# haesungpyun/seoul_tourism_recommendation_NGCF

Hardware: NVIDIA B200
Metric: ngcf_epoch_time_fwd_bwd_bpr (lower is better)
Workload: dtype f32

## Files before the change

seoul_tourism_recommendation_ngcf_b200/csrc/spmm.cu:

```cuda
#include "spmm_core.cuh"

namespace {

using namespace ngcf;

#ifndef NGCF_SPMM_THREADS
#define NGCF_SPMM_THREADS 64
#endif
constexpr int SP_THREADS = NGCF_SPMM_THREADS;
constexpr int SP_WARPS = SP_THREADS / 32;

struct TileSide {
    const TileInfo* tiles;
    const int32_t* rowptr;
    const int2* ent;
    const int32_t* row_key;
    const uint8_t* bits;
    const int2* cent;
    const int32_t* ccnt;
    float* Y;
    int64_t ldy;
};

struct SpmmArgs {
    TileSide rows, chunks;
    int n_chunk_tiles;
    const float* X;
    uint32_t ldx;
    int d;
    const float* addend;
    int64_t ld_add;
    const int32_t* slot;
    const float* gsum;
    int64_t ld_gsum;
    const int32_t* hub_of_row;
    const int32_t* hub_chunk_ptr;
    int32_t* hub_done;
    float* Yrows;
    int64_t ld_yrows;
    float drop_p;
    uint64_t seed;
    const uint64_t* seed_dev;
    int layer;
    int transposed;
    uint32_t row_off;
    unsigned long long* dbg;
    const uint32_t* tile_hubmask;
    int n_row_tiles;
    int add_mode;
    const int32_t* hub_rows;
    int n_hub;
};

__device__ __forceinline__ unsigned long long gtime_ns() {
    unsigned long long t;
    asm volatile("mov.u64 %0, %%globaltimer;" : "=l"(t));
    return t;
}
__device__ __forceinline__ void stamp_done(unsigned long long* dbg) {
    __syncthreads();
    if (threadIdx.x == 0) {
        unsigned smid;
        asm volatile("mov.u32 %0, %%smid;" : "=r"(smid));
        dbg[blockIdx.x * 4 + 2] = gtime_ns();
        dbg[blockIdx.x * 4 + 3] = smid;
    }
}

struct CtaSync {
    __device__ __forceinline__ void operator()() const { __syncthreads(); }
};

#ifndef NGCF_SPMM_CTAS
#define NGCF_SPMM_CTAS 20
#endif
template <int G>
__global__ void __launch_bounds__(SP_THREADS, NGCF_SPMM_CTAS) spmm_tile_kernel(SpmmArgs a) {
    __shared__ __align__(16) int2 ent_s[SP_TILE_ENT];
    __shared__ int rp_s[SP_TILE_ROWS + 1];
    __shared__ int hub_s[SP_TILE_ROWS];
    const int tid = threadIdx.x, lane = tid & 31, warp = tid >> 5;
    pdl_launch_dependents();
    if (a.dbg && tid == 0) a.dbg[blockIdx.x * 4 + 0] = gtime_ns();
    const bool chunk_side = (int)blockIdx.x < a.n_chunk_tiles;
    const TileSide& sd = chunk_side ? a.chunks : a.rows;
    const int t = chunk_side ? (int)blockIdx.x : (int)blockIdx.x - a.n_chunk_tiles;
    const int4 raw = *reinterpret_cast<const int4*>(sd.tiles + t);
    const TileInfo ti{raw.x, raw.y, raw.z, raw.w};
    const int nr = ti.r1 - ti.r0;
    if (tid < nr)
        hub_s[tid] = chunk_side ? a.hub_of_row[sd.row_key[ti.r0 + tid]] : (a.hub_of_row ? a.hub_of_row[ti.r0 + tid] : -1);
    pdl_wait();
    {
        DropArgs dr{a.drop_p, a.drop_p > 0.f ? ngcf_seed(a.seed, a.seed_dev) : 0ull, a.layer, a.transposed,
                    a.row_off, sd.bits};
        stage_tile<SP_THREADS>(ti, sd.rowptr, sd.ent, sd.row_key, dr, rp_s, ent_s, tid, CtaSync());
    }
    if (a.dbg && tid == 0) a.dbg[blockIdx.x * 4 + 1] = gtime_ns();

    if (chunk_side) {
        for (int i = warp; i < nr; i += SP_WARPS) {
            const int64_t chunk = ti.r0 + i;
            const int h = hub_s[i];
            if constexpr (G > 0) {
                const float4 acc = gather_row_vec<G>(ent_s, rp_s[i], rp_s[i + 1], a.X, a.ldx, a.d, lane);
                if (lane < G && lane * 4 < a.d) st_f4(sd.Y + chunk * sd.ldy + lane * 4, acc);
            } else {
                float acc[SC_MAXQ];
                gather_row_sc(ent_s, rp_s[i], rp_s[i + 1], a.X, a.ldx, a.d, lane, acc);
#pragma unroll
                for (int q = 0; q < SC_MAXQ; ++q)
                    if (lane + 32 * q < a.d) sd.Y[chunk * sd.ldy + lane + 32 * q] = acc[q];
            }
            __threadfence();
            __syncwarp();
            const int c0 = a.hub_chunk_ptr[h], c1 = a.hub_chunk_ptr[h + 1];
            int last = 0;
            if (lane == 0) last = (atomicAdd(a.hub_done + h, 1) + 1 == c1 - c0);
            last = __shfl_sync(FULL_MASK, last, 0);
            if (!last) continue;
            __threadfence();
            if (lane == 0) a.hub_done[h] = 0;
            const int64_t row = sd.row_key[chunk] ;
            const int s = a.slot ? a.slot[row] : -1;
            if constexpr (G > 0) {
                float4 sum = sum_partials_split<G>(sd.Y, c0, c1, a.d, lane);
                if (lane < G && lane * 4 < a.d) {
                    const int c = lane * 4;
                    if (a.addend) {
                        const float4 ad = ld_f4(a.addend + row * a.ld_add + c);
                        sum.x += ad.x; sum.y += ad.y; sum.z += ad.z; sum.w += ad.w;
                    }
                    if (s >= 0) {
                        const float4 gs = ld_f4(a.gsum + (int64_t)s * a.ld_gsum + c);
                        sum.x += gs.x; sum.y += gs.y; sum.z += gs.z; sum.w += gs.w;
                    }
                    st_f4(a.Yrows + row * a.ld_yrows + c, sum);
                }
            } else {
                float sum[SC_MAXQ];
                sum_partials_sc(sd.Y, c0, c1, a.d, lane, sum);
#pragma unroll
                for (int q = 0; q < SC_MAXQ; ++q) {
                    const int col = lane + 32 * q;
                    if (col < a.d) {
                        float r = sum[q];
                        if (a.addend) r += a.addend[row * a.ld_add + col];
                        if (s >= 0) r += a.gsum[(int64_t)s * a.ld_gsum + col];
                        a.Yrows[row * a.ld_yrows + col] = r;
                    }
                }
            }
        }
        if (a.dbg) stamp_done(a.dbg);
        return;
    }

    if constexpr (G > 0) {
        for (int i = warp; i < nr; i += SP_WARPS) {
            if (hub_s[i] >= 0) continue;
            const int64_t row = ti.r0 + i;
            const bool ok = lane < G && lane * 4 < a.d;
            float4 ad = make_float4(0.f, 0.f, 0.f, 0.f);
            int s = -1;
            if (ok && a.addend) ad = ld_f4(a.addend + row * a.ld_add + lane * 4);
            if (ok && a.slot) s = a.slot[row];
            float4 acc = gather_row_vec<G>(ent_s, rp_s[i], rp_s[i + 1], a.X, a.ldx, a.d, lane);
            if (ok) {
                acc.x += ad.x; acc.y += ad.y; acc.z += ad.z; acc.w += ad.w;
                if (s >= 0) {
                    const float4 gs = ld_f4(a.gsum + (int64_t)s * a.ld_gsum + lane * 4);
                    acc.x += gs.x; acc.y += gs.y; acc.z += gs.z; acc.w += gs.w;
                }
                st_f4(sd.Y + row * sd.ldy + lane * 4, acc);
            }
        }
    } else {
        for (int i = warp; i < nr; i += SP_WARPS) {
            if (hub_s[i] >= 0) continue;
            const int64_t row = ti.r0 + i;
            float acc[SC_MAXQ];
            gather_row_sc(ent_s, rp_s[i], rp_s[i + 1], a.X, a.ldx, a.d, lane, acc);
            const int s = a.slot ? a.slot[row] : -1;
#pragma unroll
            for (int q = 0; q < SC_MAXQ; ++q) {
                const int col = lane + 32 * q;
                if (col < a.d) {
                    float r = acc[q];
                    if (a.addend) r += a.addend[row * a.ld_add + col];
                    if (s >= 0) r += a.gsum[(int64_t)s * a.ld_gsum + col];
                    sd.Y[row * sd.ldy + col] = r;
                }
            }
        }
    }
    if (a.dbg) stamp_done(a.dbg);
}

__device__ __forceinline__ void red_add_f4(float* p, float4 v) {
    asm volatile("red.global.add.v4.f32 [%0], {%1, %2, %3, %4};" ::"l"(p), "f"(v.x), "f"(v.y), "f"(v.z), "f"(v.w) : "memory");
}

template <int G>
__global__ void __launch_bounds__(SP_THREADS, NGCF_SPMM_CTAS) spmm_stream_kernel(SpmmArgs a) {
    constexpr int NGRP = SP_THREADS / G;
    __shared__ __align__(16) int2 ent_s[SP_TILE_ENT];
    __shared__ __align__(16) float ysum[SP_TILE_ROWS * G * 4];
    __shared__ __align__(16) float pf[SP_THREADS * 4];
    __shared__ int rp_s[SP_TILE_ROWS + 1];
    __shared__ int first_row[NGRP];
    const int tid = threadIdx.x, lane = tid & 31, warp = tid >> 5;
    const int grp = tid / G, l = tid % G;
    pdl_launch_dependents();
    if (a.dbg && tid == 0) a.dbg[blockIdx.x * 4 + 0] = gtime_ns();
    const bool chunk_side = (int)blockIdx.x < a.n_chunk_tiles;
    const TileSide& sd = chunk_side ? a.chunks : a.rows;
    const int t = chunk_side ? (int)blockIdx.x : (int)blockIdx.x - a.n_chunk_tiles;
    const int4 raw = *reinterpret_cast<const int4*>(sd.tiles + t);
    const TileInfo ti{raw.x, raw.y, raw.z, raw.w};
    const int nr = ti.r1 - ti.r0;
    const uint32_t hubmask = (!chunk_side && a.tile_hubmask) ? a.tile_hubmask[t] : 0u;
#pragma unroll
    for (int i = tid; i < SP_TILE_ROWS * G; i += SP_THREADS) reinterpret_cast<float4*>(ysum)[i] = make_float4(0.f, 0.f, 0.f, 0.f);
    pdl_wait();
    int cnt;
    if (sd.ccnt) {
        cnt = sd.ccnt[t];
        for (int i = tid; i < cnt; i += SP_THREADS) ent_s[i] = ld_stream_i2(sd.cent + ti.e0 + i);
        __syncthreads();
    } else {
        cnt = ti.e1 - ti.e0;
        DropArgs dr{a.drop_p, a.drop_p > 0.f ? ngcf_seed(a.seed, a.seed_dev) : 0ull, a.layer, a.transposed,
                    a.row_off, sd.bits};
        stage_tile<SP_THREADS>(ti, sd.rowptr, sd.ent, sd.row_key, dr, rp_s, ent_s, tid, CtaSync());
    }
    if (a.dbg && tid == 0) a.dbg[blockIdx.x * 4 + 1] = gtime_ns();

    {
        const int per = (cnt + NGRP - 1) / NGRP;
        int j = min(grp * per, cnt);
        const int end = min(j + per, cnt);
        const char* xl = reinterpret_cast<const char*>(a.X + ((l * 4) < a.d ? l * 4 : 0));
        const uint32_t row_bytes = a.ldx * 4u;
        float* const pf_l = pf + grp * (G * 4) + l * 4;
        float* const ys_l = ysum + l * 4;
        float4 acc = make_float4(0.f, 0.f, 0.f, 0.f);
        int cur = -1, frow = -1;
        bool isfirst = true;
        auto step = [&](const int2 e, const float4 x) {
            const int lr = ent_lrow(e.x);
            if (lr != cur) {
                if (cur >= 0) {
                    st_f4(isfirst ? pf_l : ys_l + cur * (G * 4), acc);
                    if (isfirst) frow = cur;
                    isfirst = false;
                }
                acc = make_float4(0.f, 0.f, 0.f, 0.f);
                cur = lr;
            }
            const float w = __int_as_float(e.y);
            acc.x = fmaf(w, x.x, acc.x);
            acc.y = fmaf(w, x.y, acc.y);
            acc.z = fmaf(w, x.z, acc.z);
            acc.w = fmaf(w, x.w, acc.w);
        };
        for (; j + UNROLL <= end; j += UNROLL) {
            int2 e[UNROLL];
            float4 x[UNROLL];
#pragma unroll
            for (int u = 0; u < UNROLL; ++u) e[u] = ent_s[j + u];
#pragma unroll
            for (int u = 0; u < UNROLL; ++u)
                x[u] = ld_f4(reinterpret_cast<const float*>(xl + (uint64_t)ent_col(e[u].x) * row_bytes));
#pragma unroll
            for (int u = 0; u < UNROLL; ++u) step(e[u], x[u]);
        }
        if (j < end) {
            int2 e[UNROLL];
            float4 x[UNROLL];
#pragma unroll
            for (int u = 0; u < UNROLL; ++u) {
                e[u] = make_int2(0, 0);
                x[u] = make_float4(0.f, 0.f, 0.f, 0.f);
                if (j + u < end) {
                    e[u] = ent_s[j + u];
                    x[u] = ld_f4(reinterpret_cast<const float*>(xl + (uint64_t)ent_col(e[u].x) * row_bytes));
                }
            }
#pragma unroll
            for (int u = 0; u < UNROLL; ++u)
                if (j + u < end) step(e[u], x[u]);
        }
        if (cur >= 0) {
            st_f4(isfirst ? pf_l : ys_l + cur * (G * 4), acc);
            if (isfirst) frow = cur;
        }
        if (l == 0) first_row[grp] = frow;
    }
    __syncthreads();

    auto row_sum = [&](int i, int ll) {
        float4 y = ld_f4(ysum + i * (G * 4) + ll * 4);
#pragma unroll
        for (int q = 0; q < NGRP; ++q)
            if (first_row[q] == i) {
                const float4 p = ld_f4(pf + q * (G * 4) + ll * 4);
                y.x += p.x; y.y += p.y; y.z += p.z; y.w += p.w;
            }
        return y;
    };

    if (chunk_side) {
        const bool okc = l * 4 < a.d;
        for (int i = grp; i < nr; i += NGRP)
            if (okc) st_f4(sd.Y + (int64_t)(ti.r0 + i) * sd.ldy + l * 4, row_sum(i, l));
        if (a.dbg) stamp_done(a.dbg);
        return;
    }

    const bool ok = l * 4 < a.d;
    for (int i = grp; i < nr; i += NGRP) {
        if (((hubmask >> i) & 1u) || !ok) continue;
        const int64_t row = ti.r0 + i;
        float4 y = row_sum(i, l);
        const int s = a.slot ? a.slot[row] : -1;
        if (s >= 0) {
            const float4 gs = ld_f4(a.gsum + (int64_t)s * a.ld_gsum + l * 4);
            y.x += gs.x; y.y += gs.y; y.z += gs.z; y.w += gs.w;
        }
        float* dst = sd.Y + row * sd.ldy + l * 4;
        if (a.add_mode) red_add_f4(dst, y); else st_f4(dst, y);
    }
    if (a.dbg) stamp_done(a.dbg);
}

constexpr int HF_THREADS = 128;
template <int G>
__global__ void __launch_bounds__(HF_THREADS) hub_finish_kernel(SpmmArgs a) {
    constexpr int NGRP = HF_THREADS / G;
    __shared__ __align__(16) float gs[HF_THREADS * 4];
    pdl_launch_dependents();
    const int tid = threadIdx.x, g = tid / G, l = tid % G;
    const int h = blockIdx.x;
    const int c0 = a.hub_chunk_ptr[h], c1 = a.hub_chunk_ptr[h + 1];
    const int64_t row = a.hub_rows[h];
    pdl_wait();
    const bool ok = l * 4 < a.d;
    float* const dst = a.Yrows + row * a.ld_yrows + l * 4;
    float4 ad = make_float4(0.f, 0.f, 0.f, 0.f);
    int s = -1;
    if (g == 0 && ok) {
        if (a.add_mode) ad = ld_f4(dst);
        if (a.slot) s = a.slot[row];
    }
    float4 acc = make_float4(0.f, 0.f, 0.f, 0.f);
    if (ok) {
        const float* p = a.chunks.Y + l * 4;
        int c = c0 + g;
        for (; c + 3 * NGRP < c1; c += 4 * NGRP) {
            float4 x[4];
#pragma unroll
            for (int u = 0; u < 4; ++u) x[u] = __ldcg(reinterpret_cast<const float4*>(p + (int64_t)(c + u * NGRP) * a.d));
#pragma unroll
            for (int u = 0; u < 4; ++u) { acc.x += x[u].x; acc.y += x[u].y; acc.z += x[u].z; acc.w += x[u].w; }
        }
        for (; c < c1; c += NGRP) {
            const float4 x = __ldcg(reinterpret_cast<const float4*>(p + (int64_t)c * a.d));
            acc.x += x.x; acc.y += x.y; acc.z += x.z; acc.w += x.w;
        }
    }
    st_f4(gs + g * (G * 4) + l * 4, acc);
    __syncthreads();
    if (g == 0 && ok) {
        float4 sum = acc;
#pragma unroll
        for (int q = 1; q < NGRP; ++q) {
            const float4 v = ld_f4(gs + q * (G * 4) + l * 4);
            sum.x += v.x; sum.y += v.y; sum.z += v.z; sum.w += v.w;
        }
        if (a.add_mode) {
            sum.x += ad.x; sum.y += ad.y; sum.z += ad.z; sum.w += ad.w;
        }
        if (s >= 0) {
            const float4 gsv = ld_f4(a.gsum + (int64_t)s * a.ld_gsum + l * 4);
            sum.x += gsv.x; sum.y += gsv.y; sum.z += gsv.z; sum.w += gsv.w;
        }
        st_f4(dst, sum);
    }
}

struct BitsArgs {
    const TileInfo* tiles;
    const int32_t* rowptr;
    const int2* ent;
    const int32_t* row_key;
    float p;
    uint64_t seed;
    const uint64_t* seed_dev;
    int n_layers;
    uint32_t row_off;
    uint8_t* out_f;
    uint8_t* out_t;
};

constexpr int BITS_THREADS = 256;
constexpr int BITS_TILES = 8;
__global__ void __launch_bounds__(BITS_THREADS) dropout_bits_kernel(BitsArgs a, int n_tiles) {
    __shared__ int rp_s[BITS_TILES * SP_TILE_ROWS + 1];
    const int tid = threadIdx.x;
    const int t0 = blockIdx.x * BITS_TILES, t1 = min(t0 + BITS_TILES, n_tiles) - 1;
    const int4 first = *reinterpret_cast<const int4*>(a.tiles + t0);
    const int4 last = *reinterpret_cast<const int4*>(a.tiles + t1);
    const int r0 = first.x, nr = last.y - first.x, e0 = first.z, cnt = last.w - first.z;
    for (int i = tid; i <= nr; i += BITS_THREADS) rp_s[i] = a.rowptr[r0 + i] - e0;
    __syncthreads();
    const uint64_t seed = ngcf_seed(a.seed, a.seed_dev);
    for (int i = tid; i < cnt; i += BITS_THREADS) {
        const uint32_t c = ent_col(ld_stream_i2(a.ent + e0 + i).x);
        int lo = 0, hi = nr - 1;
        while (lo < hi) {
            const int mid = (lo + hi + 1) >> 1;
            if (rp_s[mid] <= i) lo = mid; else hi = mid - 1;
        }
        const uint32_t r = (uint32_t)(a.row_key ? a.row_key[r0 + lo] : r0 + lo) + a.row_off;
        if (a.out_f) a.out_f[e0 + i] = (uint8_t)node_keep_bits(a.p, seed, a.n_layers, r, c);
        if (a.out_t) a.out_t[e0 + i] = (uint8_t)node_keep_bits(a.p, seed, a.n_layers, c, r);
    }
}

struct KeyArgs {
    const TileInfo* tiles;
    const int32_t* rowptr;
    const int2* ent;
    const int32_t* row_key;
    uint32_t row_off;
    uint32_t* key_l;
    uint32_t* key_t;
};
__global__ void __launch_bounds__(BITS_THREADS) entry_keys_kernel(KeyArgs a, int n_tiles) {
    __shared__ int rp_s[BITS_TILES * SP_TILE_ROWS + 1];
    const int tid = threadIdx.x;
    const int t0 = blockIdx.x * BITS_TILES, t1 = min(t0 + BITS_TILES, n_tiles) - 1;
    const int4 first = *reinterpret_cast<const int4*>(a.tiles + t0);
    const int4 last = *reinterpret_cast<const int4*>(a.tiles + t1);
    const int r0 = first.x, nr = last.y - first.x, e0 = first.z, cnt = last.w - first.z;
    for (int i = tid; i <= nr; i += BITS_THREADS) rp_s[i] = a.rowptr[r0 + i] - e0;
    __syncthreads();
    for (int i = tid; i < cnt; i += BITS_THREADS) {
        const uint32_t c = ent_col(ld_stream_i2(a.ent + e0 + i).x);
        int lo = 0, hi = nr - 1;
        while (lo < hi) {
            const int mid = (lo + hi + 1) >> 1;
            if (rp_s[mid] <= i) lo = mid; else hi = mid - 1;
        }
        const uint32_t r = (uint32_t)(a.row_key ? a.row_key[r0 + lo] : r0 + lo) + a.row_off;
        a.key_l[e0 + i] = ngcf_node_key(r, c);
        a.key_t[e0 + i] = ngcf_node_key(c, r);
    }
}

constexpr int WS_PER = SP_TILE_ENT / 32;
static_assert(WS_PER * 32 == SP_TILE_ENT, "tile entries must be a multiple of the warp size");

struct CompactArgs {
    const TileInfo* tiles;
    const int2* ent;
    const int32_t* row_key;
    float p;
    uint64_t seed;
    const uint64_t* seed_dev;
    int n_layers;
    uint32_t row_off;
    const uint32_t* key_l;
    const uint32_t* key_t;
    int2* out_ent[2][NGCF_MAX_LAYERS];
    int32_t* out_cnt[2][NGCF_MAX_LAYERS];
};

constexpr int CW_WARPS = 4;
__global__ void __launch_bounds__(CW_WARPS * 32) compact_kernel(CompactArgs a, int n_tiles) {
    const int lane = threadIdx.x & 31;
    const int t = blockIdx.x * CW_WARPS + (threadIdx.x >> 5);
    if (t >= n_tiles) return;
    const int4 raw = *reinterpret_cast<const int4*>(a.tiles + t);
    const TileInfo ti{raw.x, raw.y, raw.z, raw.w};
    const int cnt = ti.e1 - ti.e0;
    const int K = a.n_layers;
    const bool want_l = a.out_ent[0][0] != nullptr, want_t = a.out_ent[1][0] != nullptr;
    int2 e[WS_PER];
    uint32_t kl[WS_PER], kt[WS_PER];
#pragma unroll
    for (int q = 0; q < WS_PER; ++q) {
        const int p = q * 32 + lane;
        e[q] = make_int2(0, 0);
        kl[q] = kt[q] = 0;
        if (p < cnt) {
            e[q] = ld_stream_i2(a.ent + ti.e0 + p);
            if (a.key_l) {
                if (want_l) kl[q] = a.key_l[ti.e0 + p];
                if (want_t) kt[q] = a.key_t[ti.e0 + p];
            }
        }
    }
    const uint64_t seed = ngcf_seed(a.seed, a.seed_dev);
    const uint32_t thr = ngcf_threshold16(a.p);
    uint32_t keep[WS_PER];
#pragma unroll
    for (int q = 0; q < WS_PER; ++q) {
        const int p = q * 32 + lane;
        keep[q] = 0;
        if (p < cnt) {
            if (!a.key_l) {
                const int lr = ent_lrow(e[q].x);
                const uint32_t r = (uint32_t)(a.row_key ? a.row_key[ti.r0 + lr] : ti.r0 + lr) + a.row_off;
                kl[q] = ngcf_node_key(r, ent_col(e[q].x));
                kt[q] = ngcf_node_key(ent_col(e[q].x), r);
            }
            if (want_l) keep[q] = node_keep_bits_key(thr, seed, K, kl[q]);
            if (want_t) keep[q] |= node_keep_bits_key(thr, seed, K, kt[q]) << K;
        }
    }
    const uint32_t below = (1u << lane) - 1u;
    for (int c = 0; c < 2 * K; ++c) {
        const int dir = c >= K, layer = dir ? c - K : c;
        int2* out = a.out_ent[dir][layer];
        if (!out) continue;
        int base = 0;
#pragma unroll
        for (int q = 0; q < WS_PER; ++q) {
            const bool k = (keep[q] >> c) & 1u;
            const uint32_t m = __ballot_sync(FULL_MASK, k);
            if (k) out[ti.e0 + base + __popc(m & below)] = e[q];
            base += __popc(m);
        }
        if (lane == 0) a.out_cnt[dir][layer][t] = base;
    }
}

template <int G>
int launch(const SpmmArgs& a, int n_ctas, bool stream, cudaStream_t st) {
    if (n_ctas <= 0) return NGCF_OK;
    if constexpr (G > 0) {
        if (stream) {
            NGCF_CUDA(ngcf_launch_pdl(spmm_stream_kernel<G>, dim3((unsigned)n_ctas), dim3(SP_THREADS), 0, st, a));
            NGCF_LAUNCH_OK("spmm_stream_kernel");
            if (a.n_hub > 0) {
                NGCF_CUDA(ngcf_launch_pdl(hub_finish_kernel<G>, dim3((unsigned)a.n_hub), dim3(HF_THREADS), 0, st, a));
                NGCF_LAUNCH_OK("hub_finish_kernel");
            }
            return NGCF_OK;
        }
    }
    NGCF_CUDA(ngcf_launch_pdl(spmm_tile_kernel<G>, dim3((unsigned)n_ctas), dim3(SP_THREADS), 0, st, a));
    NGCF_LAUNCH_OK("spmm_tile_kernel");
    return NGCF_OK;
}

int launch_any(const SpmmArgs& a, int n_ctas, bool vec, bool stream, cudaStream_t st) {
    if (!vec) return launch<0>(a, n_ctas, false, st);
    const int d4 = a.d / 4;
    if (d4 <= 1) return launch<1>(a, n_ctas, stream, st);
    if (d4 <= 2) return launch<2>(a, n_ctas, stream, st);
    if (d4 <= 4) return launch<4>(a, n_ctas, stream, st);
    if (d4 <= 8) return launch<8>(a, n_ctas, stream, st);
    if (d4 <= 16) return launch<16>(a, n_ctas, stream, st);
    return launch<32>(a, n_ctas, stream, st);
}

unsigned long long* g_spmm_dbg = nullptr;
unsigned long long* g_spmm_dbg_compact = nullptr;

inline bool aligned16(const void* p) { return (reinterpret_cast<uintptr_t>(p) & 15) == 0; }

}

extern "C" int ngcf_spmm_split_threshold(void) { return ngcf::SPLIT; }
extern "C" int ngcf_spmm_tile_rows(void) { return SP_TILE_ROWS; }
extern "C" int ngcf_spmm_tile_entries(void) { return SP_TILE_ENT; }

int ngcf_check_csr(const ngcf_csr* g, const char* who) {
    NGCF_REQUIRE(g != nullptr, "%s: csr descriptor is null", who);
    NGCF_REQUIRE(g->n_rows >= 0 && g->n_rows < ((int64_t)1 << 31), "%s: n_rows %lld", who, (long long)g->n_rows);
    NGCF_REQUIRE(g->n_rows == 0 || (g->rowptr && g->ent), "%s: rowptr/ent missing", who);
    NGCF_REQUIRE(g->n_hub >= 0 && g->n_chunks >= 0, "%s: negative hub counts", who);
    NGCF_REQUIRE(g->n_hub == 0 || (g->hub_of_row && g->hub_chunk_ptr && g->chunk_ptr && g->hub_ent && g->chunk_row),
                 "%s: hub arrays missing", who);
    return NGCF_OK;
}

extern "C" int ngcf_spmm(const ngcf_csr* g, const float* X, int64_t ldx, int d, const float* addend, int64_t ld_add,
                         const int32_t* slot, const float* gsum, int64_t ld_gsum, float* hub_partial, float drop_p,
                         uint64_t seed, const uint64_t* seed_dev, int layer, int transposed, int64_t row_offset,
                         const uint8_t* keep_bits, const int32_t* c_ent, const int32_t* c_cnt, float* Y, int64_t ldy,
                         void* stream) {
    int rc = ngcf_check_csr(g, "spmm");
    if (rc != NGCF_OK) return rc;
    NGCF_REQUIRE(X && Y, "spmm: null pointer");
    NGCF_REQUIRE(d > 0 && d <= NGCF_MAX_WIDTH, "spmm: width %d not in [1,%d]", d, NGCF_MAX_WIDTH);
    NGCF_REQUIRE(ldx >= d && ldy >= d && ldx < ((int64_t)1 << 31), "spmm: bad leading dimension");
    NGCF_REQUIRE(drop_p >= 0.f && drop_p < 1.f, "spmm: drop_p %f not in [0,1)", drop_p);
    NGCF_REQUIRE(layer >= 0 && layer < NGCF_MAX_LAYERS, "spmm: layer %d", layer);
    NGCF_REQUIRE(row_offset >= 0 && row_offset < ((int64_t)1 << 31), "spmm: row_offset %lld", (long long)row_offset);
    NGCF_REQUIRE(!slot || gsum, "spmm: slot given without gsum");
    NGCF_REQUIRE((c_ent == nullptr) == (c_cnt == nullptr), "spmm: c_ent and c_cnt go together");
    NGCF_REQUIRE(g->n_hub == 0 || hub_partial, "spmm: hub_partial scratch missing");
    NGCF_REQUIRE(g->n_tiles == 0 || g->tiles, "spmm: SpMM tiles missing");
    NGCF_REQUIRE(g->n_chunk_tiles == 0 || g->chunk_tiles, "spmm: chunk tiles missing");
    if (g->n_rows == 0) return NGCF_OK;
    cudaStream_t st = as_stream(stream);
    const bool vec = (d % 4 == 0) && (ldx % 4 == 0) && (ldy % 4 == 0) && aligned16(X) && aligned16(Y) &&
                     (!addend || (aligned16(addend) && ld_add % 4 == 0)) &&
                     (!slot || (aligned16(gsum) && ld_gsum % 4 == 0)) && (g->n_hub == 0 || aligned16(hub_partial));
    const bool hubs = g->n_hub > 0 && g->n_chunks > 0;
    const bool stream_k = vec && (!hubs || (g->tile_hubmask && g->hub_rows));
    NGCF_REQUIRE(stream_k || !c_ent, "spmm: compacted survivor lists need the streaming kernel (width %% 4 == 0)");
    NGCF_REQUIRE(stream_k || !hubs || g->hub_done, "spmm: hub_done counters missing");
    SpmmArgs a{};
    a.rows = TileSide{reinterpret_cast<const TileInfo*>(g->tiles), g->rowptr, reinterpret_cast<const int2*>(g->ent), nullptr,
                      keep_bits, reinterpret_cast<const int2*>(c_ent), c_cnt, Y, ldy};
    a.n_chunk_tiles = hubs ? g->n_chunk_tiles : 0;
    if (hubs)
        a.chunks = TileSide{reinterpret_cast<const TileInfo*>(g->chunk_tiles), g->chunk_ptr,
                            reinterpret_cast<const int2*>(g->hub_ent), g->chunk_row,
                            keep_bits ? keep_bits + g->rowptr_nnz : nullptr,
                            c_ent ? reinterpret_cast<const int2*>(c_ent) + g->rowptr_nnz : nullptr,
                            c_cnt ? c_cnt + g->n_tiles : nullptr, hub_partial, d};
    a.X = X; a.ldx = (uint32_t)ldx; a.d = d;
    a.addend = addend; a.ld_add = ld_add; a.slot = slot; a.gsum = gsum; a.ld_gsum = ld_gsum;
    a.drop_p = drop_p; a.seed = seed; a.seed_dev = seed_dev; a.layer = layer; a.transposed = transposed;
    a.row_off = (uint32_t)row_offset;
    a.dbg = g_spmm_dbg;
    a.hub_of_row = hubs ? g->hub_of_row : nullptr;
    a.hub_chunk_ptr = g->hub_chunk_ptr;
    a.hub_done = g->hub_done;
    a.Yrows = Y;
    a.ld_yrows = ldy;
    a.tile_hubmask = hubs ? g->tile_hubmask : nullptr;
    a.n_row_tiles = g->n_tiles;
    a.hub_rows = g->hub_rows;
    a.n_hub = hubs ? g->n_hub : 0;
    if (stream_k && addend) {
        if (addend != Y)
            NGCF_CUDA(cudaMemcpy2DAsync(Y, (size_t)ldy * sizeof(float), addend, (size_t)ld_add * sizeof(float),
                                        (size_t)d * sizeof(float), (size_t)g->n_rows, cudaMemcpyDeviceToDevice, st));
        a.add_mode = 1;
        a.addend = nullptr;
    }
    return launch_any(a, a.n_chunk_tiles + g->n_tiles, vec, stream_k, st);
}

extern "C" int ngcf_node_dropout_bits(const ngcf_csr* g, float drop_p, uint64_t seed, const uint64_t* seed_dev,
                                      int n_layers, int64_t row_offset, uint8_t* bits_as_L, uint8_t* bits_as_Lt,
                                      void* stream) {
    int rc = ngcf_check_csr(g, "node_dropout_bits");
    if (rc != NGCF_OK) return rc;
    NGCF_REQUIRE(drop_p > 0.f && drop_p < 1.f, "node_dropout_bits: drop_p %f not in (0,1)", drop_p);
    NGCF_REQUIRE(n_layers >= 1 && n_layers <= NGCF_MAX_LAYERS, "node_dropout_bits: n_layers %d", n_layers);
    NGCF_REQUIRE(bits_as_L || bits_as_Lt, "node_dropout_bits: no output");
    NGCF_REQUIRE(row_offset >= 0 && row_offset < ((int64_t)1 << 31), "node_dropout_bits: row_offset");
    cudaStream_t st = as_stream(stream);
    if (g->n_tiles > 0) {
        BitsArgs a{reinterpret_cast<const TileInfo*>(g->tiles), g->rowptr, reinterpret_cast<const int2*>(g->ent), nullptr,
                   drop_p, seed, seed_dev, n_layers, (uint32_t)row_offset, bits_as_L, bits_as_Lt};
        dropout_bits_kernel<<<(unsigned)ceil_div64(g->n_tiles, BITS_TILES), BITS_THREADS, 0, st>>>(a, g->n_tiles);
        NGCF_LAUNCH_OK("dropout_bits_kernel(rows)");
    }
    if (g->n_hub > 0 && g->n_chunk_tiles > 0) {
        BitsArgs a{reinterpret_cast<const TileInfo*>(g->chunk_tiles), g->chunk_ptr,
                   reinterpret_cast<const int2*>(g->hub_ent), g->chunk_row, drop_p, seed, seed_dev, n_layers,
                   (uint32_t)row_offset, bits_as_L ? bits_as_L + g->rowptr_nnz : nullptr,
                   bits_as_Lt ? bits_as_Lt + g->rowptr_nnz : nullptr};
        dropout_bits_kernel<<<(unsigned)ceil_div64(g->n_chunk_tiles, BITS_TILES), BITS_THREADS, 0, st>>>(a, g->n_chunk_tiles);
        NGCF_LAUNCH_OK("dropout_bits_kernel(hub chunks)");
    }
    return NGCF_OK;
}

extern "C" int ngcf_node_dropout_compact(const ngcf_csr* g, float drop_p, uint64_t seed, const uint64_t* seed_dev,
                                         int n_layers, int64_t row_offset, int32_t* const* ent_as_L_host,
                                         int32_t* const* cnt_as_L_host, int32_t* const* ent_as_Lt_host,
                                         int32_t* const* cnt_as_Lt_host, void* stream) {
    int rc = ngcf_check_csr(g, "node_dropout_compact");
    if (rc != NGCF_OK) return rc;
    NGCF_REQUIRE(drop_p > 0.f && drop_p < 1.f, "node_dropout_compact: drop_p %f not in (0,1)", drop_p);
    NGCF_REQUIRE(n_layers >= 1 && n_layers <= NGCF_MAX_LAYERS, "node_dropout_compact: n_layers %d", n_layers);
    NGCF_REQUIRE((ent_as_L_host && cnt_as_L_host) || (ent_as_Lt_host && cnt_as_Lt_host), "node_dropout_compact: no output");
    NGCF_REQUIRE((ent_as_L_host == nullptr) == (cnt_as_L_host == nullptr) &&
                 (ent_as_Lt_host == nullptr) == (cnt_as_Lt_host == nullptr), "node_dropout_compact: ent/cnt go together");
    NGCF_REQUIRE(row_offset >= 0 && row_offset < ((int64_t)1 << 31), "node_dropout_compact: row_offset");
    for (int k = 0; k < n_layers; ++k) {
        NGCF_REQUIRE(!ent_as_L_host || (ent_as_L_host[k] && cnt_as_L_host[k]), "node_dropout_compact: null L output %d", k);
        NGCF_REQUIRE(!ent_as_Lt_host || (ent_as_Lt_host[k] && cnt_as_Lt_host[k]), "node_dropout_compact: null L^T output %d", k);
    }
    cudaStream_t st = as_stream(stream);
    for (int pass = 0; pass < 2; ++pass) {
        const int n_tiles = pass ? g->n_chunk_tiles : g->n_tiles;
        if (n_tiles <= 0 || (pass && g->n_hub == 0)) continue;
        CompactArgs a{};
        a.tiles = reinterpret_cast<const TileInfo*>(pass ? g->chunk_tiles : g->tiles);
        a.ent = reinterpret_cast<const int2*>(pass ? g->hub_ent : g->ent);
        a.row_key = pass ? g->chunk_row : nullptr;
        a.p = drop_p; a.seed = seed; a.seed_dev = seed_dev; a.n_layers = n_layers; a.row_off = (uint32_t)row_offset;
        const size_t e_off = pass ? (size_t)g->rowptr_nnz : 0, t_off = pass ? (size_t)g->n_tiles : 0;
        if (g->key_l && g->key_t && g->key_row_offset == row_offset) {
            a.key_l = g->key_l + e_off;
            a.key_t = g->key_t + e_off;
        }
        for (int k = 0; k < n_layers; ++k) {
            if (ent_as_L_host) {
                a.out_ent[0][k] = reinterpret_cast<int2*>(ent_as_L_host[k]) + e_off;
                a.out_cnt[0][k] = cnt_as_L_host[k] + t_off;
            }
            if (ent_as_Lt_host) {
                a.out_ent[1][k] = reinterpret_cast<int2*>(ent_as_Lt_host[k]) + e_off;
                a.out_cnt[1][k] = cnt_as_Lt_host[k] + t_off;
            }
        }
        compact_kernel<<<(unsigned)ceil_div64(n_tiles, CW_WARPS), CW_WARPS * 32, 0, st>>>(a, n_tiles);
        NGCF_LAUNCH_OK(pass ? "compact_kernel(hub chunks)" : "compact_kernel(rows)");
    }
    return NGCF_OK;
}

extern "C" int ngcf_debug_spmm_timeline(unsigned long long* dev_buf_or_null) {
    g_spmm_dbg = dev_buf_or_null;
    return NGCF_OK;
}
extern "C" int ngcf_debug_compact_timeline(unsigned long long* dev_buf_or_null) {
    g_spmm_dbg_compact = dev_buf_or_null;
    return NGCF_OK;
}

extern "C" int ngcf_entry_keys(const ngcf_csr* g, int64_t row_offset, uint32_t* key_l, uint32_t* key_t, void* stream) {
    int rc = ngcf_check_csr(g, "entry_keys");
    if (rc != NGCF_OK) return rc;
    NGCF_REQUIRE(key_l && key_t, "entry_keys: null output");
    NGCF_REQUIRE(row_offset >= 0 && row_offset < ((int64_t)1 << 31), "entry_keys: row_offset");
    cudaStream_t st = as_stream(stream);
    if (g->n_tiles > 0) {
        KeyArgs a{reinterpret_cast<const TileInfo*>(g->tiles), g->rowptr, reinterpret_cast<const int2*>(g->ent), nullptr,
                  (uint32_t)row_offset, key_l, key_t};
        entry_keys_kernel<<<(unsigned)ceil_div64(g->n_tiles, BITS_TILES), BITS_THREADS, 0, st>>>(a, g->n_tiles);
        NGCF_LAUNCH_OK("entry_keys_kernel(rows)");
    }
    if (g->n_hub > 0 && g->n_chunk_tiles > 0) {
        KeyArgs a{reinterpret_cast<const TileInfo*>(g->chunk_tiles), g->chunk_ptr, reinterpret_cast<const int2*>(g->hub_ent),
                  g->chunk_row, (uint32_t)row_offset, key_l + g->rowptr_nnz, key_t + g->rowptr_nnz};
        entry_keys_kernel<<<(unsigned)ceil_div64(g->n_chunk_tiles, BITS_TILES), BITS_THREADS, 0, st>>>(a, g->n_chunk_tiles);
        NGCF_LAUNCH_OK("entry_keys_kernel(hub chunks)");
    }
    return NGCF_OK;
}
```

Before: 0.4962.

## Process multiple SpMM tiles per CTA in the streaming kernel

The streaming SpMM kernel now loops over up to SP_MAX_T tiles per CTA. The tiles-per-CTA count comes from the resident CTA count found with the occupancy API. When no dropout masking is needed, a COPY variant copies entries straight from precompacted or raw storage and skips the masking stage, and the shared-memory row sums are zeroed as they are read so they can be reused for the next tile. This is meant to cut CTA launch and scheduling overhead and the per-tile setup cost, at the price of less parallelism and possible load imbalance when tiles vary in size.

```diff
diff --git a/seoul_tourism_recommendation_ngcf_b200/csrc/spmm.cu b/seoul_tourism_recommendation_ngcf_b200/csrc/spmm.cu
--- a/seoul_tourism_recommendation_ngcf_b200/csrc/spmm.cu
+++ b/seoul_tourism_recommendation_ngcf_b200/csrc/spmm.cu
@@ -50,6 +50,8 @@
     int add_mode;
     const int32_t* hub_rows;
     int n_hub;
+    int n_tiles_total;
+    int tiles_per_cta;
 };
 
 __device__ __forceinline__ unsigned long long gtime_ns() {
@@ -200,136 +202,172 @@
 __device__ __forceinline__ void red_add_f4(float* p, float4 v) {
     asm volatile("red.global.add.v4.f32 [%0], {%1, %2, %3, %4};" ::"l"(p), "f"(v.x), "f"(v.y), "f"(v.z), "f"(v.w) : "memory");
 }
-
-template <int G>
+#ifndef NGCF_SPMM_MAX_T
+#define NGCF_SPMM_MAX_T 4
+#endif
+constexpr int SP_MAX_T = NGCF_SPMM_MAX_T;
+
+template <int G, bool COPY>
 __global__ void __launch_bounds__(SP_THREADS, NGCF_SPMM_CTAS) spmm_stream_kernel(SpmmArgs a) {
     constexpr int NGRP = SP_THREADS / G;
     __shared__ __align__(16) int2 ent_s[SP_TILE_ENT];
     __shared__ __align__(16) float ysum[SP_TILE_ROWS * G * 4];
     __shared__ __align__(16) float pf[SP_THREADS * 4];
+    __shared__ __align__(16) int4 rec_s[SP_MAX_T];
+    __shared__ uint32_t hm_s[SP_MAX_T];
+    __shared__ int cnt_s[SP_MAX_T];
+    __shared__ int nt_s;
     __shared__ int rp_s[SP_TILE_ROWS + 1];
     __shared__ int first_row[NGRP];
-    const int tid = threadIdx.x, lane = tid & 31, warp = tid >> 5;
+    const int tid = threadIdx.x;
     const int grp = tid / G, l = tid % G;
     pdl_launch_dependents();
     if (a.dbg && tid == 0) a.dbg[blockIdx.x * 4 + 0] = gtime_ns();
-    const bool chunk_side = (int)blockIdx.x < a.n_chunk_tiles;
-    const TileSide& sd = chunk_side ? a.chunks : a.rows;
-    const int t = chunk_side ? (int)blockIdx.x : (int)blockIdx.x - a.n_chunk_tiles;
-    const int4 raw = *reinterpret_cast<const int4*>(sd.tiles + t);
-    const TileInfo ti{raw.x, raw.y, raw.z, raw.w};
-    const int nr = ti.r1 - ti.r0;
-    const uint32_t hubmask = (!chunk_side && a.tile_hubmask) ? a.tile_hubmask[t] : 0u;
+    const int T = COPY ? a.tiles_per_cta : 1;
+    const int g0 = (int)blockIdx.x * T;
+    const int nt = min(T, a.n_tiles_total - g0);
+    if (tid == 0) nt_s = nt;
+    if (tid < nt) {
+        const int g = g0 + tid;
+        const bool cs = g < a.n_chunk_tiles;
+        const int t = cs ? g : g - a.n_chunk_tiles;
+        rec_s[tid] = *reinterpret_cast<const int4*>((cs ? a.chunks.tiles : a.rows.tiles) + t);
+        hm_s[tid] = (!cs && a.tile_hubmask) ? a.tile_hubmask[t] : 0u;
+    }
 #pragma unroll
     for (int i = tid; i < SP_TILE_ROWS * G; i += SP_THREADS) reinterpret_cast<float4*>(ysum)[i] = make_float4(0.f, 0.f, 0.f, 0.f);
+    __syncthreads();
     pdl_wait();
-    int cnt;
-    if (sd.ccnt) {
-        cnt = sd.ccnt[t];
-        for (int i = tid; i < cnt; i += SP_THREADS) ent_s[i] = ld_stream_i2(sd.cent + ti.e0 + i);
+    if (COPY && tid < nt) {
+        const int g = g0 + tid;
+        const bool cs = g < a.n_chunk_tiles;
+        const int32_t* ccnt = cs ? a.chunks.ccnt : a.rows.ccnt;
+        cnt_s[tid] = ccnt ? ccnt[cs ? g : g - a.n_chunk_tiles] : rec_s[tid].w - rec_s[tid].z;
+    }
+
+    for (int k = 0; k < nt_s; ++k) {
         __syncthreads();
-    } else {
-        cnt = ti.e1 - ti.e0;
-        DropArgs dr{a.drop_p, a.drop_p > 0.f ? ngcf_seed(a.seed, a.seed_dev) : 0ull, a.layer, a.transposed,
-                    a.row_off, sd.bits};
-        stage_tile<SP_THREADS>(ti, sd.rowptr, sd.ent, sd.row_key, dr, rp_s, ent_s, tid, CtaSync());
-    }
-    if (a.dbg && tid == 0) a.dbg[blockIdx.x * 4 + 1] = gtime_ns();
-
-    {
-        const int per = (cnt + NGRP - 1) / NGRP;
-        int j = min(grp * per, cnt);
-        const int end = min(j + per, cnt);
-        const char* xl = reinterpret_cast<const char*>(a.X + ((l * 4) < a.d ? l * 4 : 0));
-        const uint32_t row_bytes = a.ldx * 4u;
-        float* const pf_l = pf + grp * (G * 4) + l * 4;
-        float* const ys_l = ysum + l * 4;
-        float4 acc = make_float4(0.f, 0.f, 0.f, 0.f);
-        int cur = -1, frow = -1;
-        bool isfirst = true;
-        auto step = [&](const int2 e, const float4 x) {
-            const int lr = ent_lrow(e.x);
-            if (lr != cur) {
-                if (cur >= 0) {
-                    st_f4(isfirst ? pf_l : ys_l + cur * (G * 4), acc);
-                    if (isfirst) frow = cur;
-                    isfirst = false;
+        int cnt;
+        {
+            const bool cs = g0 + k < a.n_chunk_tiles;
+            const TileSide& sd = cs ? a.chunks : a.rows;
+            const int4 raw = rec_s[k];
+            const TileInfo ti{raw.x, raw.y, raw.z, raw.w};
+            if constexpr (COPY) {
+                cnt = cnt_s[k];
+                const int2* src = (sd.ccnt ? sd.cent : sd.ent) + ti.e0;
+                for (int i = tid; i < cnt; i += SP_THREADS) ent_s[i] = ld_stream_i2(src + i);
+                __syncthreads();
+            } else {
+                cnt = ti.e1 - ti.e0;
+                DropArgs dr{a.drop_p, a.drop_p > 0.f ? ngcf_seed(a.seed, a.seed_dev) : 0ull, a.layer, a.transposed,
+                            a.row_off, sd.bits};
+                stage_tile<SP_THREADS>(ti, sd.rowptr, sd.ent, sd.row_key, dr, rp_s, ent_s, tid, CtaSync());
+            }
+        }
+        if (a.dbg && tid == 0 && k == 0) a.dbg[blockIdx.x * 4 + 1] = gtime_ns();
+
+        {
+            const int per = (cnt + NGRP - 1) / NGRP;
+            int j = min(grp * per, cnt);
+            const int end = min(j + per, cnt);
+            const char* xl = reinterpret_cast<const char*>(a.X + ((l * 4) < a.d ? l * 4 : 0));
+            const uint32_t row_bytes = a.ldx * 4u;
+            float* const pf_l = pf + grp * (G * 4) + l * 4;
+            float* const ys_l = ysum + l * 4;
+            float4 acc = make_float4(0.f, 0.f, 0.f, 0.f);
+            int cur = -1, frow = -1;
+            bool isfirst = true;
+            auto step = [&](const int2 e, const float4 x) {
+                const int lr = ent_lrow(e.x);
+                if (lr != cur) {
+                    if (cur >= 0) {
+                        st_f4(isfirst ? pf_l : ys_l + cur * (G * 4), acc);
+                        if (isfirst) frow = cur;
+                        isfirst = false;
+                    }
+                    acc = make_float4(0.f, 0.f, 0.f, 0.f);
+                    cur = lr;
                 }
-                acc = make_float4(0.f, 0.f, 0.f, 0.f);
-                cur = lr;
-            }
-            const float w = __int_as_float(e.y);
-            acc.x = fmaf(w, x.x, acc.x);
-            acc.y = fmaf(w, x.y, acc.y);
-            acc.z = fmaf(w, x.z, acc.z);
-            acc.w = fmaf(w, x.w, acc.w);
+                const float w = __int_as_float(e.y);
+                acc.x = fmaf(w, x.x, acc.x);
+                acc.y = fmaf(w, x.y, acc.y);
+                acc.z = fmaf(w, x.z, acc.z);
+                acc.w = fmaf(w, x.w, acc.w);
+            };
+            for (; j + UNROLL <= end; j += UNROLL) {
+                int2 e[UNROLL];
+                float4 x[UNROLL];
+#pragma unroll
+                for (int u = 0; u < UNROLL; ++u) e[u] = ent_s[j + u];
+#pragma unroll
+                for (int u = 0; u < UNROLL; ++u)
+                    x[u] = ld_f4(reinterpret_cast<const float*>(xl + (uint64_t)ent_col(e[u].x) * row_bytes));
+#pragma unroll
+                for (int u = 0; u < UNROLL; ++u) step(e[u], x[u]);
+            }
+            if (j < end) {
+                int2 e[UNROLL];
+                float4 x[UNROLL];
+#pragma unroll
+                for (int u = 0; u < UNROLL; ++u) {
+                    e[u] = make_int2(0, 0);
+                    x[u] = make_float4(0.f, 0.f, 0.f, 0.f);
+                    if (j + u < end) {
+                        e[u] = ent_s[j + u];
+                        x[u] = ld_f4(reinterpret_cast<const float*>(xl + (uint64_t)ent_col(e[u].x) * row_bytes));
+                    }
+                }
+#pragma unroll
+                for (int u = 0; u < UNROLL; ++u)
+                    if (j + u < end) step(e[u], x[u]);
+            }
+            if (cur >= 0) {
+                st_f4(isfirst ? pf_l : ys_l + cur * (G * 4), acc);
+                if (isfirst) frow = cur;
+            }
+            if (l == 0) first_row[grp] = frow;
+        }
+        __syncthreads();
+        const bool chunk_side = g0 + k < a.n_chunk_tiles;
+        const TileSide& sd = chunk_side ? a.chunks : a.rows;
+        const int r0 = rec_s[k].x, nr = rec_s[k].y - r0;
+
+        auto row_sum = [&](int i, int ll) {
+            float4* ys = reinterpret_cast<float4*>(ysum + i * (G * 4) + ll * 4);
+            float4 y = *ys;
+            *ys = make_float4(0.f, 0.f, 0.f, 0.f);
+#pragma unroll
+            for (int q = 0; q < NGRP; ++q)
+                if (first_row[q] == i) {
+                    const float4 p = ld_f4(pf + q * (G * 4) + ll * 4);
+                    y.x += p.x; y.y += p.y; y.z += p.z; y.w += p.w;
+                }
+            return y;
         };
-        for (; j + UNROLL <= end; j += UNROLL) {
-            int2 e[UNROLL];
-            float4 x[UNROLL];
-#pragma unroll
-            for (int u = 0; u < UNROLL; ++u) e[u] = ent_s[j + u];
-#pragma unroll
-            for (int u = 0; u < UNROLL; ++u)
-                x[u] = ld_f4(reinterpret_cast<const float*>(xl + (uint64_t)ent_col(e[u].x) * row_bytes));
-#pragma unroll
-            for (int u = 0; u < UNROLL; ++u) step(e[u], x[u]);
-        }
-        if (j < end) {
-            int2 e[UNROLL];
-            float4 x[UNROLL];
-#pragma unroll
-            for (int u = 0; u < UNROLL; ++u) {
-                e[u] = make_int2(0, 0);
-                x[u] = make_float4(0.f, 0.f, 0.f, 0.f);
-                if (j + u < end) {
-                    e[u] = ent_s[j + u];
-                    x[u] = ld_f4(reinterpret_cast<const float*>(xl + (uint64_t)ent_col(e[u].x) * row_bytes));
-                }
-            }
-#pragma unroll
-            for (int u = 0; u < UNROLL; ++u)
-                if (j + u < end) step(e[u], x[u]);
-        }
-        if (cur >= 0) {
-            st_f4(isfirst ? pf_l : ys_l + cur * (G * 4), acc);
-            if (isfirst) frow = cur;
-        }
-        if (l == 0) first_row[grp] = frow;
-    }
-    __syncthreads();
-
-    auto row_sum = [&](int i, int ll) {
-        float4 y = ld_f4(ysum + i * (G * 4) + ll * 4);
-#pragma unroll
-        for (int q = 0; q < NGRP; ++q)
-            if (first_row[q] == i) {
-                const float4 p = ld_f4(pf + q * (G * 4) + ll * 4);
-                y.x += p.x; y.y += p.y; y.z += p.z; y.w += p.w;
-            }
-        return y;
-    };
-
-    if (chunk_side) {
-        const bool okc = l * 4 < a.d;
-        for (int i = grp; i < nr; i += NGRP)
-            if (okc) st_f4(sd.Y + (int64_t)(ti.r0 + i) * sd.ldy + l * 4, row_sum(i, l));
-        if (a.dbg) stamp_done(a.dbg);
-        return;
-    }
-
-    const bool ok = l * 4 < a.d;
-    for (int i = grp; i < nr; i += NGRP) {
-        if (((hubmask >> i) & 1u) || !ok) continue;
-        const int64_t row = ti.r0 + i;
-        float4 y = row_sum(i, l);
-        const int s = a.slot ? a.slot[row] : -1;
-        if (s >= 0) {
-            const float4 gs = ld_f4(a.gsum + (int64_t)s * a.ld_gsum + l * 4);
-            y.x += gs.x; y.y += gs.y; y.z += gs.z; y.w += gs.w;
-        }
-        float* dst = sd.Y + row * sd.ldy + l * 4;
-        if (a.add_mode) red_add_f4(dst, y); else st_f4(dst, y);
+
+        const bool ok = l * 4 < a.d;
+        if (chunk_side) {
+            for (int i = grp; i < nr; i += NGRP) {
+                const float4 y = row_sum(i, l);
+                if (ok) st_f4(sd.Y + (int64_t)(r0 + i) * sd.ldy + l * 4, y);
+            }
+            continue;
+        }
+
+        const uint32_t hubmask = hm_s[k];
+        for (int i = grp; i < nr; i += NGRP) {
+            float4 y = row_sum(i, l);
+            if (((hubmask >> i) & 1u) || !ok) continue;
+            const int64_t row = r0 + i;
+            const int s_row = a.slot ? a.slot[row] : -1;
+            if (s_row >= 0) {
+                const float4 gs = ld_f4(a.gsum + (int64_t)s_row * a.ld_gsum + l * 4);
+                y.x += gs.x; y.y += gs.y; y.z += gs.z; y.w += gs.w;
+            }
+            float* dst = sd.Y + row * sd.ldy + l * 4;
+            if (a.add_mode) red_add_f4(dst, y); else st_f4(dst, y);
+        }
     }
     if (a.dbg) stamp_done(a.dbg);
 }
@@ -537,13 +575,43 @@
     }
 }
 
+template <int G, bool COPY>
+int stream_resident_ctas(int* out) {
+    static int cached[64] = {};
+    int dev = 0;
+    NGCF_CUDA(cudaGetDevice(&dev));
+    int& c = cached[dev & 63];
+    if (c == 0) {
+        int per_sm = 0;
+        NGCF_CUDA(cudaOccupancyMaxActiveBlocksPerMultiprocessor(&per_sm, spmm_stream_kernel<G, COPY>, SP_THREADS, 0));
+        NGCF_REQUIRE(per_sm > 0, "spmm: spmm_stream_kernel<%d, %d> cannot be resident", G, (int)COPY);
+        c = ngcf_num_sms() * per_sm;
+    }
+    *out = c;
+    return NGCF_OK;
+}
+
+template <int G, bool COPY>
+int launch_stream(SpmmArgs a, int n_tiles, cudaStream_t st) {
+    int resident = 0;
+    const int rc = stream_resident_ctas<G, COPY>(&resident);
+    if (rc != NGCF_OK) return rc;
+    a.n_tiles_total = n_tiles;
+    a.tiles_per_cta = COPY ? std::max(1, std::min(n_tiles / resident, SP_MAX_T)) : 1;
+    const int n_ctas = (int)ceil_div64(n_tiles, a.tiles_per_cta);
+    NGCF_CUDA(ngcf_launch_pdl(spmm_stream_kernel<G, COPY>, dim3((unsigned)n_ctas), dim3(SP_THREADS), 0, st, a));
+    NGCF_LAUNCH_OK("spmm_stream_kernel");
+    return NGCF_OK;
+}
+
 template <int G>
-int launch(const SpmmArgs& a, int n_ctas, bool stream, cudaStream_t st) {
-    if (n_ctas <= 0) return NGCF_OK;
+int launch(SpmmArgs a, int n_tiles, bool stream, cudaStream_t st) {
+    if (n_tiles <= 0) return NGCF_OK;
     if constexpr (G > 0) {
         if (stream) {
-            NGCF_CUDA(ngcf_launch_pdl(spmm_stream_kernel<G>, dim3((unsigned)n_ctas), dim3(SP_THREADS), 0, st, a));
-            NGCF_LAUNCH_OK("spmm_stream_kernel");
+            const bool copy = a.rows.ccnt || (a.drop_p == 0.f && !a.rows.bits);
+            const int rc = copy ? launch_stream<G, true>(a, n_tiles, st) : launch_stream<G, false>(a, n_tiles, st);
+            if (rc != NGCF_OK) return rc;
             if (a.n_hub > 0) {
                 NGCF_CUDA(ngcf_launch_pdl(hub_finish_kernel<G>, dim3((unsigned)a.n_hub), dim3(HF_THREADS), 0, st, a));
                 NGCF_LAUNCH_OK("hub_finish_kernel");
@@ -551,20 +619,20 @@
             return NGCF_OK;
         }
     }
-    NGCF_CUDA(ngcf_launch_pdl(spmm_tile_kernel<G>, dim3((unsigned)n_ctas), dim3(SP_THREADS), 0, st, a));
+    NGCF_CUDA(ngcf_launch_pdl(spmm_tile_kernel<G>, dim3((unsigned)n_tiles), dim3(SP_THREADS), 0, st, a));
     NGCF_LAUNCH_OK("spmm_tile_kernel");
     return NGCF_OK;
 }
 
-int launch_any(const SpmmArgs& a, int n_ctas, bool vec, bool stream, cudaStream_t st) {
-    if (!vec) return launch<0>(a, n_ctas, false, st);
+int launch_any(const SpmmArgs& a, int n_tiles, bool vec, bool stream, cudaStream_t st) {
+    if (!vec) return launch<0>(a, n_tiles, false, st);
     const int d4 = a.d / 4;
-    if (d4 <= 1) return launch<1>(a, n_ctas, stream, st);
-    if (d4 <= 2) return launch<2>(a, n_ctas, stream, st);
-    if (d4 <= 4) return launch<4>(a, n_ctas, stream, st);
-    if (d4 <= 8) return launch<8>(a, n_ctas, stream, st);
-    if (d4 <= 16) return launch<16>(a, n_ctas, stream, st);
-    return launch<32>(a, n_ctas, stream, st);
+    if (d4 <= 1) return launch<1>(a, n_tiles, stream, st);
+    if (d4 <= 2) return launch<2>(a, n_tiles, stream, st);
+    if (d4 <= 4) return launch<4>(a, n_tiles, stream, st);
+    if (d4 <= 8) return launch<8>(a, n_tiles, stream, st);
+    if (d4 <= 16) return launch<16>(a, n_tiles, stream, st);
+    return launch<32>(a, n_tiles, stream, st);
 }
 
 unsigned long long* g_spmm_dbg = nullptr;
```

New measurement: 0.5213, median of 6. +5.1%, slower.
